# Hitenze/Preconditioned_Additive_Gaussian_Processes_with_Fourier_Acceleration

Hardware: AMD Instinct MI355X
Metric: kernel matvecs/sec + PCG wall-time to 1e-6, n=1e6 d=32 additive, 1/2/4/8 GPU (higher is better)
Workload: dtype f64; 1 GPU; additive NFFT matvec, n=1000000, d=32, 32 x 1-D windows, Gaussian f=1 l=1 mu=0.01 (BASELINE configs[2]); n=1000000, d=32, nwindows=32, parallelism=single

## Files before the change

preconditioned_additive_gaussian_processes_with_fourier_acceleration_amd/csrc/internal.h:

```cpp
#pragma once

#include <hip/hip_runtime.h>

#include <cstdint>
#include <memory>
#include <utility>
#include <string>
#include <vector>

#include "../../include/nfft4gp_amd.h"

namespace nfft4gp_amd {

constexpr int kNos = 64;
constexpr int kBand = 32;
constexpr int kM = 4;
constexpr int kTaps = 2 * kM + 2;
constexpr int kDeg = 7;
constexpr int kNC = kDeg + 1;
constexpr int kR = 16;
constexpr int kWave = 64;
constexpr int kPad = 32;
constexpr int kMaxBlock = 4096 - kPad;

// ... 135 lines not shown
   std::vector<double> comp_sigma;
   int kernel = 0;
   double f = 1.0, l = 1.0, mu = 0.0;
   double weight = 1.0;
   double diag = 1.0;
   int B = kMaxBlock, CG = 3, ngroups = 0, nblocks = 0;
   int rec = 5;
   int spread_variant = -1;
   int spread_fold = 1;
   bool det = false;
   double* d_hb = nullptr;
   int nparts = 0;
   DevLayout dl;
   double* d_part = nullptr;
   double* d_w = nullptr;
   double* d_wd = nullptr;
   double* d_H = nullptr;
   double* d_Hd = nullptr;
   double* d_C = nullptr;
   double* d_dot_part = nullptr;
   unsigned int* d_dot_ticket = nullptr;
   double* d_part2 = nullptr;
   double* d_gsum = nullptr;
   double* d_H2 = nullptr;
   double* d_xs = nullptr;
   double* d_ys = nullptr;
   MdPlan md;
   bool timing = false;
   hipEvent_t* kev = nullptr;
   double ms[3] = {0, 0, 0};
   long long cnt[3] = {0, 0, 0};
};

int upload_tap_coeffs();
int launch_spread(const AdditivePlan& P, const double* d_x, double* d_part, hipStream_t stream);
int launch_grid(const AdditivePlan& P, const double* d_part, int nparts, int grad, hipStream_t stream);
int launch_spread_grid(AdditivePlan& P, const double* d_x, int grad, hipStream_t stream);
int launch_grid_from_sum(const AdditivePlan& P, const double* d_gridsum, int grad, hipStream_t stream);
constexpr int kPeerInline = 8;
struct PeerArgs {
   char* const* bufs = nullptr;
   char* inl[kPeerInline] = {};
   char* own = nullptr;
   int world = 0;
   unsigned int epoch = 0;
   unsigned int* err = nullptr;
   long long slot_doubles = 0;
   long long spin = 0;
};
int launch_reduce_parts(const AdditivePlan& P, const double* d_part, double* d_gridsum, hipStream_t stream,
                        const PeerArgs* A = nullptr);
int launch_shard_finish_split(const AdditivePlan& P, const double* d_gridsum, double alpha, const double* d_x,
                              double beta, double* d_y, int S, hipStream_t stream, const PeerArgs* A = nullptr,
                              const double* d_part = nullptr);
int launch_peer_grid(const AdditivePlan& P, const PeerArgs& A, const double* d_part, hipStream_t stream);
int launch_peer_sum(const AdditivePlan& P, const PeerArgs& A, double* d_grid, hipStream_t stream);
int launch_interp(const AdditivePlan& P, int grad, double alpha, const double* d_x, double beta, double* d_y,
                  hipStream_t stream, double* d_dot = nullptr);
int launch_interp_blocks(const AdditivePlan& P, double alpha, const double* d_x, double beta, double* d_y, int b0,
                         int b1, hipStream_t stream);
int launch_matvec2(AdditivePlan& P, double alpha, const double* x0, const double* x1, double beta, double* y0,
                   double* y1, hipStream_t stream);
int pick_spread_variant(const AdditivePlan& P);
bool grid_atomic(const AdditivePlan& P);
int pick_interp_threads(const AdditivePlan& P);
bool pick_interp_hl(const AdditivePlan& P);
int pick_hl_slots(const AdditivePlan& P);
int pick_interp2_threads();
int additive_matvec_multi(void* str, int nv, double alpha, const double* const* X, double beta, double* const* Y);
int additive_matvec_dot(void* str, const double* d_x, double* d_y, double* d_dot);
AdditivePlan* additive_plan_of(void* str);
bool additive_fused_dot_ok(void* str);

struct NysDev {
   int n = 0, k = 0;
   double eta = 0.0;
   double* U = nullptr;
   float* Uf = nullptr;
   double* s = nullptr;
   double* w = nullptr;
   double* part = nullptr;
   int nblk = 0;
   double setup_ms[4] = {0.0, 0.0, 0.0, 0.0};
   std::vector<double> hs;
   bool grad = false;
   double f2 = 0.0;
   double *Kall = nullptr, *dU = nullptr, *G = nullptr, *Gt = nullptr, *GdKG = nullptr, *D = nullptr;
   double *vk = nullptr, *vn = nullptr;
};
void nys_free(NysDev* N);
constexpr int kNysRows = 2048;
// ... 158 lines not shown
```

preconditioned_additive_gaussian_processes_with_fourier_acceleration_amd/csrc/nfft_api.cpp:

```cpp
#include <dlfcn.h>
#include <hip/hip_runtime.h>

#include <array>
#include <algorithm>
#include <atomic>
#include <chrono>
#include <thread>
#include <cmath>
#include <cstdio>
#include <cstdlib>
#include <cstring>
#include <mutex>
#include <vector>

#include "internal.h"
#include "reduce.hpp"

using namespace nfft4gp_amd;

namespace nfft4gp_amd {

namespace {
std::recursive_mutex g_rand_mu;
int g_rand_depth = 0;
// ... 52 lines not shown
      ok = cnt > 0 ? 1 : 0;
   }
   return ok;
}

bool is_device_ptr(const void* p)
{
   if (!p) return false;
   hipPointerAttribute_t attr;
   hipError_t e = hipPointerGetAttributes(&attr, p);
   if (e != hipSuccess) {
      (void)hipGetLastError();
      return false;
   }
   return attr.type == hipMemoryTypeDevice || attr.type == hipMemoryTypeManaged;
}

}

namespace {

struct TimingRec {
   std::array<hipEvent_t, 6> ev;
};

struct PlanExt {
   AdditivePlan P;
   std::vector<TimingRec> pending;
   std::vector<TimingRec> pool;
};

struct SingleAdj {
   str_adj pub{};
   double sigma_pub = 0.0;
   nfft4gp_kernel* owner = nullptr;
   int dim = 1;
   int max_n = 0;
   std::vector<double> data;
   PlanExt* plan = nullptr;
};

void dfree(void* p)
{
   if (p) (void)hipFree(p);
}

// ... 8 lines not shown
   dfree(P.d_part);
   dfree(P.d_part2);
   dfree(P.d_H2);
   dfree(P.d_dot_part);
   dfree(P.d_dot_ticket);
   P.d_part2 = P.d_H2 = nullptr;
   P.d_part = nullptr;
   P.d_dot_part = nullptr;
   P.d_dot_ticket = nullptr;
}

void free_plan(PlanExt* E)
{
   if (!E) return;
   AdditivePlan& P = E->P;
   free_layout(P);
   md_free(P);
   dfree(P.d_w);
   dfree(P.d_wd);
   dfree(P.d_H);
   dfree(P.d_Hd);
   dfree(P.d_hb);
   dfree(P.d_gsum);
   dfree(P.d_C);
   dfree(P.d_xs);
   dfree(P.d_ys);
   for (auto& r : E->pending)
      for (auto e : r.ev) (void)hipEventDestroy(e);
   for (auto& r : E->pool)
      for (auto e : r.ev) (void)hipEventDestroy(e);
   delete E;
}

template <class T, class A>
int upload(T** dptr, const std::vector<T, A>& h)
{
   if (*dptr) {
      (void)hipFree(*dptr);
      *dptr = nullptr;
   }
   if (h.empty()) return 0;
   NFFT4GP_HIP_CHECK(hipMalloc((void**)dptr, sizeof(T) * h.size()));
   NFFT4GP_HIP_CHECK(hipMemcpy(*dptr, h.data(), sizeof(T) * h.size(), hipMemcpyHostToDevice));
   return 0;
}

// ... 35 lines not shown
{
   const int ng = P.n_global;
   RawVec<uint32_t> qc((size_t)P.nw * P.n);
   P.comp_scale.assign(P.nw, 1.0);
   P.comp_centre.assign(P.nw, 0.0);
   std::vector<double> xs;
   if (std::any_of(P.comp_dims.begin(), P.comp_dims.end(), [](int d) { return d != 1; })) {
      std::vector<std::vector<double>> xsc(P.nw);
      for (int c = 0; c < P.nw; c++) {
         const double* col = buffer + (size_t)c * ng * P.dw;
         P.comp_scale[c] = centre_and_scale(col, ng, P.comp_dims[c], xsc[c]);
         if (P.comp_scale[c] < 0.0) {
            fprintf(stderr, "nfft4gp_amd: all points of window %d coincide (radius 0); the reference's scaling "
                            "0.25/radius (nfft_interface.c:190) is undefined there.\n", c);
            return -1;
         }
      }
      if (md_build_points(P, xsc)) return -1;
      P.points_ready = true;
      return 0;
   }
   const auto t0 = std::chrono::steady_clock::now();
   std::atomic<int> next{0};
   auto work = [&]() {
      std::vector<double> xw;
      for (int c = next++; c < P.nw; c = next++) {
         const double* col = buffer + (size_t)c * ng * P.dw;
         P.comp_scale[c] = centre_and_scale(col, ng, 1, xw, &P.comp_centre[c]);
         if (P.comp_scale[c] < 0.0) continue;
         for (int j = 0; j < P.n; j++) qc[(size_t)c * P.n + j] = quantize(xw[(size_t)P.row_begin + j]);
      }
   };
   {
      const int nt = std::max(1, std::min({16, P.nw, (int)std::thread::hardware_concurrency()}));
      std::vector<std::thread> th;
      for (int t = 1; t < nt; t++) th.emplace_back(work);
      work();
      for (auto& t : th) t.join();
   }
   for (int c = 0; c < P.nw; c++)
      if (P.comp_scale[c] < 0.0) {
         fprintf(stderr,
                 "nfft4gp_amd: all points of window %d coincide (radius 0); the reference's scaling "
                 "0.25/radius (nfft_interface.c:190) is undefined there.\n", c);
         return -1;
      }
   const auto t1 = std::chrono::steady_clock::now();
   free_layout(P);
   hipStream_t s = current_stream();
   uint32_t* d_qc = nullptr;
   NFFT4GP_HIP_CHECK(hipMalloc((void**)&d_qc, sizeof(uint32_t) * std::max<size_t>(1, qc.size())));
   NFFT4GP_HIP_CHECK(hipMemcpyAsync(d_qc, qc.data(), sizeof(uint32_t) * qc.size(), hipMemcpyHostToDevice, s));
   const auto t2 = std::chrono::steady_clock::now();
   const int rc_dev = build_layout_dev(d_qc, P.n, P.nw, P.B, P.CG, P, s, P.rec);
   (void)hipStreamSynchronize(s);
   (void)hipFree(d_qc);
   if (rc_dev) {
      Layout L;
      build_layout(qc.data(), P.n, P.nw, P.B, P.CG, L, P.rec);
      P.ngroups = L.ngroups;
      P.nblocks = L.nblocks;
      free_layout(P);
      if (upload(&P.dl.meta, L.meta) || upload(&P.dl.lo, L.lo) || upload(&P.dl.q, L.q) ||
          upload(&P.dl.tile_off, L.tile_off) || upload(&P.dl.cmax, L.cmax))
         return -1;
      P.dl.ntiles = L.ntiles;
      P.dl.bytes = L.meta.size() * 2 + L.lo.size() * 4 + L.q.size() * 4 + L.tile_off.size() * 4;
   }
   if (getenv("NFFT4GP_AMD_VERBOSE")) {
// ... 45 lines not shown
      P.comp_sigma[c] = sig;
      bhat_1d(kernel == 0 ? 0 : 2, sig, bh);
      bhat_1d(kernel == 0 ? 1 : 3, sig, bhd);
      const double dscale = (kernel == 0) ? 2.0 * sc * std::sqrt(2.0) / sig : sc / sig;
      circulant_1d(bh, P.weight, w.data() + (size_t)c * kNos);
      circulant_1d(bhd, P.weight * dscale, wd.data() + (size_t)c * kNos);
   }
   if (upload(&P.d_w, w) || upload(&P.d_wd, wd)) return -1;
   return 0;
}

TimingRec get_rec(PlanExt* E)
{
   if (!E->pool.empty()) {
      TimingRec r = E->pool.back();
      E->pool.pop_back();
      return r;
   }
   TimingRec r;
   for (auto& e : r.ev) (void)hipEventCreate(&e);
   return r;
}

int plan_apply_dev(PlanExt* E, int grad, double alpha, const double* d_x, double beta, double* d_y)
{
   AdditivePlan& P = E->P;
   hipStream_t s = current_stream();
   TimingRec rec;
   if (P.timing) {
      rec = get_rec(E);
      if (!P.md.on) P.kev = rec.ev.data();
   }
   const bool mdt = P.timing && P.md.on;
   int rc = 0;
   if (mdt) (void)hipEventRecord(rec.ev[0], s);
   if (P.md.on) {
      rc = md_spread(P, d_x, P.md.d_grid, s);
      if (mdt) {
         (void)hipEventRecord(rec.ev[1], s);
         (void)hipEventRecord(rec.ev[2], s);
      }
      if (!rc) rc = md_grid(P, P.md.d_grid, grad, s);
   } else {
      rc = launch_spread_grid(P, d_x, grad, s);
   }
   if (mdt) {
      (void)hipEventRecord(rec.ev[3], s);
      (void)hipEventRecord(rec.ev[4], s);
   }
   if (!rc)
      rc = P.md.on ? md_interp(P, grad, alpha, d_x, beta, d_y, s) : launch_interp(P, grad, alpha, d_x, beta, d_y, s);
   if (mdt) (void)hipEventRecord(rec.ev[5], s);
   P.kev = nullptr;
   if (P.timing) {
      if (rc)
         E->pool.push_back(rec);
      else
         E->pending.push_back(rec);
   }
   return rc ? -1 : 0;
}

int plan_apply(PlanExt* E, int n, int grad, double alpha, const double* x, double beta, double* y)
{
   AdditivePlan& P = E->P;
   if (!P.points_ready) {
      fprintf(stderr, "nfft4gp_amd: matvec called before the kernel setup (func_kernel) call.\n");
      return -1;
   }
   if (n != P.n) {
      fprintf(stderr, "nfft4gp_amd: matvec size %d does not match the handle (%d).\n", n, P.n);
      return -1;
   }
// ... 76 lines not shown
{
   P.B = default_block(P.n);
   {
      const int nw = std::max(P.nw, 1), nblocks = std::max(1, (P.n + P.B - 1) / P.B);
      auto pick = [&](int cgmax) {
         const int ngroups = (nw + cgmax - 1) / cgmax;
         P.CG = (nw + ngroups - 1) / ngroups;
         return ngroups;
      };
      if ((long long)pick(4) * nblocks < 384) pick(3);
   }
   if (const char* e = getenv("NFFT4GP_AMD_BLOCK")) {
      const int v = atoi(e);
      if (v >= 256) P.B = std::min(v, kMaxBlock) & ~15;
   }
   if (const char* e = getenv("NFFT4GP_AMD_CG")) {
      const int v = atoi(e);
      if (v >= 1 && v <= 64) P.CG = v;
   }
   if (const char* e = getenv("NFFT4GP_AMD_SPREAD_VARIANT")) P.spread_variant = atoi(e);
   if (const char* e = getenv("NFFT4GP_AMD_SPREAD_FOLD")) P.spread_fold = atoi(e) != 0;
   if (const char* e = getenv("NFFT4GP_AMD_DET")) P.det = atoi(e) != 0;
   if (const char* e = getenv("NFFT4GP_AMD_PRECISION")) P.rec = atoi(e) == 32 ? 4 : 5;
}

void* additive_create(double* data, int n_global, int ldim, int d, int* windows, int nwindows, int dwindows, int rb,
                      int re)
{
   nfft4gp_kernel* kd = kernel_struct_create(3 * n_global);
   kd->_iparams[0] = nwindows;
   kd->_iparams[1] = dwindows;
   int skip_window = 1;
   kd->_iparams[2] = 0;
   while (skip_window < dwindows && windows[nwindows * dwindows - skip_window] < 0) {
      skip_window++;
      kd->_iparams[2]++;
   }
   kd->_ibufferp = (int**)malloc(sizeof(int*));
   kd->_ibufferp[0] = windows;
   kd->_buffer = (double*)malloc(sizeof(double) * (size_t)n_global * nwindows * dwindows);
   kd->_own_buffer = 1;
   PlanExt* E = new PlanExt();
   AdditivePlan& P = E->P;
   P.n_global = n_global;
   P.row_begin = rb;
   P.row_end = re;
// ... 26 lines not shown

}

namespace nfft4gp_amd {
bool additive_fused_dot_ok(void* str)
{
   PlanExt* E = additive_plan(str);
   if (!E || !E->P.points_ready) return false;
   const AdditivePlan& P = E->P;
   if (P.row_begin != 0 || P.row_end != P.n_global) return false;
   return P.md.on || P.nblocks <= kRedMaxBlocks;
}

int additive_matvec_dot(void* str, const double* d_x, double* d_y, double* d_dot)
{
   PlanExt* E = additive_plan(str);
   if (!E || !E->P.points_ready) return -1;
   AdditivePlan& P = E->P;
   hipStream_t s = current_stream();
   if (P.md.on) {
      if (md_spread(P, d_x, P.md.d_grid, s) || md_grid(P, P.md.d_grid, 0, s)) return -1;
      return md_interp(P, 0, 1.0, d_x, 0.0, d_y, s, d_dot);
   }
   if (launch_spread_grid(P, d_x, 0, s)) return -1;
   return launch_interp(P, 0, 1.0, d_x, 0.0, d_y, s, d_dot);
}
}

namespace nfft4gp_amd {
int additive_matvec_multi(void* str, int nv, double alpha, const double* const* X, double beta, double* const* Y)
{
   PlanExt* E = additive_plan(str);
   if (!E || !E->P.points_ready) return -1;
   AdditivePlan& P = E->P;
   if (P.row_begin != 0 || P.row_end != P.n_global) return -1;
   hipStream_t s = current_stream();
   int v = 0;
   if (!P.md.on && !P.timing)
      for (; v + 1 < nv; v += 2)
         if (launch_matvec2(P, alpha, X[v], X[v + 1], beta, Y[v], Y[v + 1], s)) return -1;
   for (; v < nv; v++)
      if (plan_apply_dev(E, 0, alpha, X[v], beta, Y[v])) return -1;
   return 0;
}

int additive_matvec_chunked(void* str, double alpha, const double* d_x, double* d_y, int nchunks,
// ... 231 lines not shown
void Nfft4GPAdditiveNFFTKernelFree(void* str)
{
   if (!str) return;
   free_plan(additive_plan(str));
   ((nfft4gp_kernel*)str)->_external = NULL;
   Nfft4GPKernelParamFree(str);
}

double* Nfft4GPNFFTAppendData(double* X1, int n1, int ldim1, int d, double* X2, int n2, int ldim2)
{
   double* X = (double*)malloc(sizeof(double) * (size_t)(n1 + n2) * d);
   for (int i = 0; i < d; i++) {
      memcpy(X + (size_t)i * (n1 + n2), X1 + (size_t)i * ldim1, sizeof(double) * n1);
      memcpy(X + (size_t)i * (n1 + n2) + n1, X2 + (size_t)i * ldim2, sizeof(double) * n2);
   }
   return X;
}

int Nfft4GPAmdAdditiveLayoutInfo(void* str, long long* out, int nout)
{
   PlanExt* E = additive_plan(str);
   if (!E || !out) return -1;
   const AdditivePlan& P = E->P;
   long long v[16] = {P.n, P.nw, P.B, P.nblocks, P.dl.ntiles, P.dl.ntiles * kWave * kR, kR, P.CG, P.ngroups,
                      (long long)P.dl.bytes, pick_spread_variant(P), grid_atomic(P), pick_interp_threads(P),
                      pick_interp_hl(P), pick_hl_slots(P), pick_interp2_threads()};
   for (int i = 0; i < nout && i < 16; i++) out[i] = v[i];
   return 0;
}

int Nfft4GPAmdSetPrecision(void* str, int bits)
{
   PlanExt* E = additive_plan(str);
   if (!E || (bits != 32 && bits != 64)) {
      fprintf(stderr, "nfft4gp_amd: Nfft4GPAmdSetPrecision needs an additive handle and bits 32 or 64\n");
      return -1;
   }
   AdditivePlan& P = E->P;
   const int rec = bits == 32 ? 4 : 5;
   if (rec == P.rec) return 0;
   (void)hipStreamSynchronize(current_stream());
   P.rec = rec;
   if (!P.points_ready || P.md.on) return 0;
   const double* buffer = ((nfft4gp_kernel*)str)->_buffer;
   P.points_ready = false;
   if (plan_build_points(P, buffer)) return -1;
   return plan_setup(P, buffer, P.kernel, P.f, P.l, P.mu);
}

int Nfft4GPAmdSetDeterministic(void* str, int on)
// ... 10 lines not shown
   PlanExt* E = additive_plan(str);
   if (!E) return -1;
   E->P.timing = enable != 0;
   if (enable) {
      (void)hipStreamSynchronize(current_stream());
      for (auto& r : E->pending) E->pool.push_back(r);
      E->pending.clear();
      for (int i = 0; i < 3; i++) {
         E->P.ms[i] = 0;
         E->P.cnt[i] = 0;
      }
   }
   return 0;
}

int Nfft4GPAmdTimingQuery(void* str, double* ms, long long* cnt)
{
   PlanExt* E = additive_plan(str);
   if (!E) return -1;
   AdditivePlan& P = E->P;
   for (auto& r : E->pending) {
      NFFT4GP_HIP_CHECK(hipEventSynchronize(r.ev[5]));
      for (int i = 0; i < 3; i++) {
         float t = 0.f;
         NFFT4GP_HIP_CHECK(hipEventElapsedTime(&t, r.ev[2 * i], r.ev[2 * i + 1]));
         P.ms[i] += t;
         P.cnt[i]++;
      }
      E->pool.push_back(r);
   }
   E->pending.clear();
   for (int i = 0; i < 3; i++) {
      if (ms) ms[i] = P.ms[i];
      if (cnt) cnt[i] = P.cnt[i];
   }
   return 0;
}

int Nfft4GPAmdKernelBench(void* str, int which, int grad, int reps, const double* x, double* y, double* ms_avg)
{
   PlanExt* E = additive_plan(str);
   if (!E || !E->P.points_ready || reps <= 0 || !ms_avg) return -1;
   AdditivePlan& P = E->P;
   if (!is_device_ptr(x) || !is_device_ptr(y)) {
      fprintf(stderr, "nfft4gp_amd: Nfft4GPAmdKernelBench needs device vectors\n");
      return -1;
// ... 311 lines not shown
```

preconditioned_additive_gaussian_processes_with_fourier_acceleration_amd/csrc/nfft_kernels.hip:

```cpp
#include <hip/hip_ext.h>
#include <hip/hip_runtime.h>

#include <algorithm>
#include <cmath>
#include <cstdio>
#include <vector>

#include "internal.h"
#include "reduce.hpp"

namespace nfft4gp_amd {

constexpr int kGridThreads = 1024;
constexpr int kMomStride = kNC + 1;
constexpr int kMomWin = kNC * kNos + 4;
template <int MOMT>
__host__ __device__ constexpr int mom_doubles_per_window()
{
   return MOMT ? kMomWin : kNos * kMomStride;
}
template <int MOMT>
__device__ __forceinline__ int mom_index(int cl, int cell, int d)
{
   return MOMT ? cl * kMomWin + d * kNos + cell : (cl * kNos + cell) * kMomStride + d;
// ... 141 lines not shown
   for (int ks = 0; ks < 2; ks++)
#pragma unroll
      for (int cb = 0; cb < 4; cb++) bm[ks][cb] = mrow[(4 * ks + k) * kNos + 16 * cb + i];
#pragma unroll
   for (int cb = 0; cb < 4; cb++) {
      f64x4 acc = {0.0, 0.0, 0.0, 0.0};
      acc = __builtin_amdgcn_mfma_f64_16x16x4f64(a[0], bm[0][cb], acc, 0, 0, 0);
      acc = __builtin_amdgcn_mfma_f64_16x16x4f64(a[1], bm[1][cb], acc, 0, 0, 0);
      mrow[k * kNos + 16 * cb + i] = acc[0];
      mrow[(4 + k) * kNos + 16 * cb + i] = acc[1];
      if (k < kTaps - 8) grow89[k * kNos + 16 * cb + i] = acc[2];
   }
   __builtin_amdgcn_fence(__ATOMIC_RELEASE, "wavefront");
   __builtin_amdgcn_wave_barrier();
   __builtin_amdgcn_fence(__ATOMIC_ACQUIRE, "wavefront");
   double v = 0.0;
#pragma unroll
   for (int tp = 0; tp < kTaps; tp++) {
      const int cell = (lane + kM - tp) & (kNos - 1);
      v += tp < 8 ? mrow[tp * kNos + cell] : grow89[(tp - 8) * kNos + cell];
   }
   return v;
}

template <int THREADS, bool TIMELINE = false, int MOMT = 1, bool DET = false, int REC = 5, bool PIPE = false>
__global__ __launch_bounds__(THREADS, 6) void k_spread(const uint16_t* __restrict__ meta,
                                                      const uint32_t* __restrict__ lo,
                                                      const uint32_t* __restrict__ qarr,
                                                      const int* __restrict__ tile_off, const int* __restrict__ cmax,
                                                      const double* __restrict__ x, int n, int B, int nblocks,
                                                      int ngroups, int CG, int nw, double* __restrict__ part,
                                                      double* __restrict__ gsum, int fold)
{
   extern __shared__ __attribute__((aligned(16))) double smem[];
   const int Bp = B + kPad;
   double* s_alpha = smem;
   double* s_mom = smem + Bp;
   uint32_t* s_red = reinterpret_cast<uint32_t*>(s_mom + CG * mom_doubles_per_window<MOMT>());

   const int xcd = blockIdx.x & 7;
   const int rest = blockIdx.x >> 3;
   const int g = rest % ngroups;
   const int b = (rest / ngroups) * 8 + xcd;
   if (b >= nblocks) return;
   if (TIMELINE) stamp(0);

// ... 686 lines not shown
      if (t + nwaves < t1) load_tile<REC>(cur, meta, lo, qarr, t + nwaves, lane);
   }
   for (; g < ngroups; g++) leave(g);
   __syncthreads();

   const double ff = f * f;
#pragma unroll
   for (int k = 0; k < kEpMax; k++) {
      if (!ep_regs) break;
      const int j = tid + k * THREADS;
      if (j >= nloc) break;
      const double v = ff * (s_y[j] + mu * xe[k]);
      y[(size_t)base + j] = (beta == 0.0) ? alpha * v : fma(beta, ye[k], alpha * v);
   }
   if (!ep_regs) {
      for (int j = tid; j < nloc; j += THREADS) {
         const size_t gj = (size_t)base + j;
         const double v = ff * (s_y[j] + mu * x[gj]);
         y[gj] = (beta == 0.0) ? alpha * v : fma(beta, y[gj], alpha * v);
      }
   }
}


template <int THREADS, bool DET = false, int REC = 5>
__global__ __launch_bounds__(THREADS) void k_interp2(const uint16_t* __restrict__ meta,
                                                     const uint32_t* __restrict__ lo,
                                                     const uint32_t* __restrict__ qarr,
                                                     const int* __restrict__ tile_off, const double* __restrict__ H,
                                                     size_t h_rs, const double* __restrict__ x0,
                                                     const double* __restrict__ x1, double* __restrict__ y0,
                                                     double* __restrict__ y1, int n, int B, int ngroups, double alpha,
                                                     double beta, double f, double mu, const double* __restrict__ hb,
                                                     int nw)
{
   extern __shared__ __attribute__((aligned(16))) double smem[];
   const int Bp = B + kPad;
   double* s_y0 = smem;
   double* s_y1 = smem + Bp;
   const int b = blockIdx.x;
   const int tid = threadIdx.x;
   const int base = b * B;
   const int nloc = min(B, n - base);
   const int lane = tid & 63;
   const int wave = tid >> 6;
   constexpr int nwaves = THREADS / 64;
// ... 129 lines not shown
static InterpFn interp_fn(bool grad, bool dot, bool small, bool det, int rec)
{
   if (rec == 4) return small ? interp_fn_t<512, 4>(grad, dot, det) : interp_fn_t<kInterpThreads, 4>(grad, dot, det);
   return small ? interp_fn_t<512, 5>(grad, dot, det) : interp_fn_t<kInterpThreads, 5>(grad, dot, det);
}
constexpr int kInterp2Threads = 1024;
typedef void (*Interp2Fn)(const uint16_t*, const uint32_t*, const uint32_t*, const int*, const double*, size_t,
                          const double*, const double*, double*, double*, int, int, int, double, double, double, double,
                          const double*, int);
template <int REC>
static Interp2Fn interp2_fn_t(bool det, bool small)
{
   if (small) return det ? k_interp2<512, true, REC> : k_interp2<512, false, REC>;
   return det ? k_interp2<kInterp2Threads, true, REC> : k_interp2<kInterp2Threads, false, REC>;
}
static Interp2Fn interp2_fn(bool det, bool small, int rec)
{
   return rec == 4 ? interp2_fn_t<4>(det, small) : interp2_fn_t<5>(det, small);
}
typedef void (*InterpPartFn)(const uint16_t*, const uint32_t*, const uint32_t*, const int*, const double*, double*, int,
                             int, int, int, double);
static InterpPartFn interp_part_fn(int rec) { return rec == 4 ? k_interp_part<512, 4> : k_interp_part<512, 5>; }

static bool static_lds_zero(const void* fn)
{
   hipFuncAttributes a;
   if (hipFuncGetAttributes(&a, fn) != hipSuccess) return false;
   return a.sharedSizeBytes == 0;
}

typedef void (*InterpHlFn)(const uint16_t*, const uint32_t*, const uint32_t*, const int*, const double*, const double*,
                           double*, int, int, int, int, int, double, double, double, double, const double*, int);
static InterpHlFn interp_hl_fn(bool small, bool det, int rec)
{
   if (rec == 4)
      return small ? (det ? k_interp_hl<512, true, 4> : k_interp_hl<512, false, 4>)
                   : (det ? k_interp_hl<1024, true, 4> : k_interp_hl<1024, false, 4>);
   return small ? (det ? k_interp_hl<512, true, 5> : k_interp_hl<512, false, 5>)
                : (det ? k_interp_hl<1024, true, 5> : k_interp_hl<1024, false, 5>);
}
bool pick_interp_hl(const AdditivePlan& P)
{
   static const int v = getenv("NFFT4GP_AMD_INTERP_HL") ? atoi(getenv("NFFT4GP_AMD_INTERP_HL")) : -1;
   return (v < 0 ? P.dl.bytes > kInfinityCacheBytes : v != 0) && P.ngroups >= 1;
}
int pick_interp_threads(const AdditivePlan& P)
// ... 9 lines not shown
   return ns;
}
int pick_interp2_threads()
{
   static const int forced = getenv("NFFT4GP_AMD_INTERP2_THREADS") ? atoi(getenv("NFFT4GP_AMD_INTERP2_THREADS")) : 0;
   return forced == 512 ? 512 : kInterp2Threads;
}

static std::vector<const void*> interp_kernels()
{
   std::vector<const void*> v;
   for (int sm = 0; sm < 2; sm++)
      for (int det = 0; det < 2; det++)
         for (int rec = 4; rec <= 5; rec++) v.push_back((const void*)interp_hl_fn(sm, det, rec));
   for (int g = 0; g < 2; g++)
      for (int d = 0; d < 2; d++)
         for (int sm = 0; sm < 2; sm++)
            for (int det = 0; det < 2; det++)
               for (int rec = 4; rec <= 5; rec++) v.push_back((const void*)interp_fn(g, d && !g, sm, det, rec));
   for (int det = 0; det < 2; det++)
      for (int sm = 0; sm < 2; sm++)
         for (int rec = 4; rec <= 5; rec++) v.push_back((const void*)interp2_fn(det, sm, rec));
   for (int rec = 4; rec <= 5; rec++) v.push_back((const void*)interp_part_fn(rec));
   return v;
}

static void raise_lds_limit_once()
{
   static const bool raised = []() {
      for (const auto& byrec : kSpreadFns)
         for (const auto& bydet : byrec)
            for (const SpreadFn f : bydet)
               (void)hipFuncSetAttribute((const void*)f, hipFuncAttributeMaxDynamicSharedMemorySize, (int)kMaxDynamicLds);
      for (const void* f : interp_kernels())
         (void)hipFuncSetAttribute(f, hipFuncAttributeMaxDynamicSharedMemorySize, (int)kMaxDynamicLds);
      (void)hipGetLastError();
      return true;
   }();
   (void)raised;
}

static bool abs_lds_ok()
{
   static const bool ok = [] {
      std::vector<const void*> v = interp_kernels();
      for (const auto& byrec : kSpreadFns)
         for (const auto& bydet : byrec)
            for (const SpreadFn f : bydet) v.push_back((const void*)f);
      for (const void* f : v)
         if (!static_lds_zero(f)) return false;
      return true;
   }();
   if (!ok) fprintf(stderr, "nfft4gp_amd: a matvec kernel has static LDS; its absolute LDS addressing would be wrong\n");
   return ok;
}

static int launch_spread_to(const AdditivePlan& P, const double* d_x, double* d_part, double* d_gsum,
                            hipStream_t stream)
{
   if (P.dl.ntiles == 0 || P.n == 0) return 0;
   raise_lds_limit_once();
   if (!abs_lds_ok()) return -1;
   const SpreadFn fn = spread_fn(P);
   const int gridx = ((P.nblocks + 7) / 8) * 8 * P.ngroups;
   launch_ev(fn, dim3(gridx), dim3(kSpreadThreads), spread_lds_bytes(P), stream, P.kev ? P.kev + 0 : nullptr,
             P.dl.meta, P.dl.lo, P.dl.q, P.dl.tile_off, (const int*)P.dl.cmax, d_x, P.n, P.B, P.nblocks, P.ngroups,
             P.CG, P.nw, d_part, d_gsum, P.spread_fold);
   NFFT4GP_HIP_CHECK(hipGetLastError());
   return 0;
}

// ... 101 lines not shown
   if (P.n == 0) return 0;
   raise_lds_limit_once();
   if (!abs_lds_ok()) return -1;
   if (d_dot && (grad || P.nblocks > kRedMaxBlocks)) {
      fprintf(stderr, "nfft4gp_amd: fused matvec-dot needs a plain matvec and <= %d blocks\n", kRedMaxBlocks);
      return -1;
   }
   const bool small = pick_interp_threads(P) == 512;
   if (!grad && !d_dot && pick_interp_hl(P)) {
      const int ns = pick_hl_slots(P);
      launch_ev(interp_hl_fn(small, P.det, P.rec), dim3(P.nblocks), dim3(small ? 512 : kInterpThreads),
                hl_lds_bytes(P.B, P.CG, P.ngroups, ns), stream, P.kev ? P.kev + 4 : nullptr, P.dl.meta, P.dl.lo,
                P.dl.q, P.dl.tile_off, (const double*)P.d_H, d_x, d_y, P.n, P.B, P.ngroups, P.CG, P.nw, alpha, beta,
                P.f, P.mu * P.diag, (const double*)P.d_hb, ns);
      NFFT4GP_HIP_CHECK(hipGetLastError());
      return 0;
   }
   const InterpFn fn = interp_fn(grad, d_dot != nullptr, small, P.det, P.rec);
   launch_ev(fn, dim3(P.nblocks), dim3(small ? 512 : kInterpThreads), interp_lds_bytes(P, grad), stream,
             P.kev ? P.kev + 4 : nullptr, P.dl.meta, P.dl.lo, P.dl.q, P.dl.tile_off, (const double*)P.d_H,
             (const double*)P.d_Hd, d_x, d_y, P.n, P.B, P.ngroups, alpha, beta, P.f, P.mu * P.diag, P.diag,
             P.d_dot_part, P.d_dot_ticket, d_dot, (const double*)P.d_hb, P.nw);
   NFFT4GP_HIP_CHECK(hipGetLastError());
   return 0;
}

int launch_interp_blocks(const AdditivePlan& P, double alpha, const double* d_x, double beta, double* d_y, int b0,
                         int b1, hipStream_t stream)
{
   if (P.n == 0 || b1 <= b0) return 0;
   raise_lds_limit_once();
   if (!abs_lds_ok()) return -1;
   const size_t off = (size_t)b0 * P.B;
   hipLaunchKernelGGL(interp_fn(false, false, false, P.det, P.rec), dim3(b1 - b0), dim3(kInterpThreads),
                      interp_lds_bytes(P, 0), stream, P.dl.meta, P.dl.lo, P.dl.q, P.dl.tile_off + (size_t)b0 * P.ngroups,
                      (const double*)P.d_H, (const double*)P.d_Hd, d_x + off, d_y + off, P.n - (int)off, P.B, P.ngroups,
                      alpha, beta, P.f, P.mu * P.diag, P.diag, (double*)nullptr, (unsigned int*)nullptr,
                      (double*)nullptr, (const double*)P.d_hb, P.nw);
   NFFT4GP_HIP_CHECK(hipGetLastError());
   return 0;
}

int launch_matvec2(AdditivePlan& P, double alpha, const double* x0, const double* x1, double beta, double* y0,
                   double* y1, hipStream_t stream)
{
   if (P.n == 0) return 0;
// ... 23 lines not shown
```

preconditioned_additive_gaussian_processes_with_fourier_acceleration_amd/nfft.py:

```python
from __future__ import annotations

import ctypes as C

import numpy as np

from . import _lib

GAUSSIAN = 0
MATERN12 = 1


def _ptr(a):
    if isinstance(a, np.ndarray):
        if not a.flags.c_contiguous or a.dtype != np.float64:
            raise ValueError("numpy vectors must be C-contiguous float64")
        return a.ctypes.data, False
    if not a.is_contiguous() or str(a.dtype) != "torch.float64":
        raise ValueError("torch vectors must be contiguous float64")
    return a.data_ptr(), a.is_cuda


def _numel(a) -> int:
    return int(a.size) if isinstance(a, np.ndarray) else int(a.numel())

# ... 117 lines not shown
            raise RuntimeError("shard spread failed")
        return grid

    def shard_grid_size(self) -> int:
        return int(_lib.lib().Nfft4GPAmdShardGridSize(self.h))

    def shard_finish(self, grid, x_local, alpha=1.0, beta=0.0, y_local=None, grad=False):
        _check_len("x_local", x_local, self.n)
        if y_local is None:
            y_local = _empty_like(x_local, (3 if grad else 1) * self.n)
        _check_len("y_local", y_local, (3 if grad else 1) * self.n)
        size = self.shard_grid_size()
        if size < 0:
            raise RuntimeError("run the kernel setup before shard_finish")
        _check_len("grid", grid, size, exact=False)
        gp, _ = _ptr(grid)
        xp, _ = _ptr(x_local)
        yp, _ = _ptr(y_local)
        if _lib.lib().Nfft4GPAmdShardFinish(self.h, gp, int(grad), float(alpha), xp, float(beta), yp) != 0:
            raise RuntimeError("shard finish failed")
        return y_local

    def layout_info(self) -> dict:
        out = (C.c_longlong * 16)()
        _lib.lib().Nfft4GPAmdAdditiveLayoutInfo(self.h, out, 16)
        keys = ["n", "nwindows", "block", "nblocks", "ntiles", "slots", "R", "comps_per_group", "ngroups",
                "layout_bytes", "spread_variant", "grid_atomic", "interp_threads", "interp_hl", "hl_slots",
                "interp2_threads"]
        return dict(zip(keys, [int(v) for v in out]))

    def set_deterministic(self, on: bool = True):
        if _lib.lib().Nfft4GPAmdSetDeterministic(self.h, int(bool(on))) != 0:
            raise RuntimeError("Nfft4GPAmdSetDeterministic failed")

    def set_precision(self, bits: int):
        if _lib.lib().Nfft4GPAmdSetPrecision(self.h, int(bits)) != 0:
            raise RuntimeError("Nfft4GPAmdSetPrecision failed")

    def timing(self, enable: bool):
        _lib.lib().Nfft4GPAmdTimingEnable(self.h, int(enable))

    def timing_query(self):
        ms = (C.c_double * 3)()
        cnt = (C.c_longlong * 3)()
        _lib.lib().Nfft4GPAmdTimingQuery(self.h, ms, cnt)
        names = ["spread", "grid", "interp"]
        return {nm: (ms[i], int(cnt[i])) for i, nm in enumerate(names)}

    KERNELS = ("spread", "grid", "interp")

    def kernel_bench(self, kernel: str, x, y, reps: int = 50, grad: bool = False) -> float:
# ... 90 lines not shown
```

Measured before the change: 14360 matvecs/s.

## Fuse grid circulant stage into interpolation kernel with double-buffered grid sums

```diff
diff --git a/preconditioned_additive_gaussian_processes_with_fourier_acceleration_amd/csrc/internal.h b/preconditioned_additive_gaussian_processes_with_fourier_acceleration_amd/csrc/internal.h
--- a/preconditioned_additive_gaussian_processes_with_fourier_acceleration_amd/csrc/internal.h
+++ b/preconditioned_additive_gaussian_processes_with_fourier_acceleration_amd/csrc/internal.h
@@ -181,6 +181,10 @@
    unsigned int* d_dot_ticket = nullptr;
    double* d_part2 = nullptr;
    double* d_gsum = nullptr;
+   int fused_grid = -1;
+   bool cells33 = false;
+   double* d_hsum = nullptr;
+   int hsum_par = 0;
    double* d_H2 = nullptr;
    double* d_xs = nullptr;
    double* d_ys = nullptr;
@@ -226,6 +230,9 @@
 bool pick_interp_hl(const AdditivePlan& P);
 int pick_hl_slots(const AdditivePlan& P);
 int pick_interp2_threads();
+bool pick_fused_grid(const AdditivePlan& P);
+int launch_matvec_fused(AdditivePlan& P, double alpha, const double* d_x, double beta, double* d_y, hipStream_t stream,
+                        double* d_dot = nullptr);
 int additive_matvec_multi(void* str, int nv, double alpha, const double* const* X, double beta, double* const* Y);
 int additive_matvec_dot(void* str, const double* d_x, double* d_y, double* d_dot);
 AdditivePlan* additive_plan_of(void* str);
diff --git a/preconditioned_additive_gaussian_processes_with_fourier_acceleration_amd/csrc/nfft_api.cpp b/preconditioned_additive_gaussian_processes_with_fourier_acceleration_amd/csrc/nfft_api.cpp
--- a/preconditioned_additive_gaussian_processes_with_fourier_acceleration_amd/csrc/nfft_api.cpp
+++ b/preconditioned_additive_gaussian_processes_with_fourier_acceleration_amd/csrc/nfft_api.cpp
@@ -98,6 +98,7 @@
 
 struct TimingRec {
    std::array<hipEvent_t, 6> ev;
+   bool grid = true;
 };
 
 struct PlanExt {
@@ -152,6 +153,7 @@
    dfree(P.d_Hd);
    dfree(P.d_hb);
    dfree(P.d_gsum);
+   dfree(P.d_hsum);
    dfree(P.d_C);
    dfree(P.d_xs);
    dfree(P.d_ys);
@@ -233,13 +235,20 @@
    }
    const auto t0 = std::chrono::steady_clock::now();
    std::atomic<int> next{0};
+   std::atomic<int> outside33{0};
    auto work = [&]() {
       std::vector<double> xw;
       for (int c = next++; c < P.nw; c = next++) {
          const double* col = buffer + (size_t)c * ng * P.dw;
          P.comp_scale[c] = centre_and_scale(col, ng, 1, xw, &P.comp_centre[c]);
          if (P.comp_scale[c] < 0.0) continue;
-         for (int j = 0; j < P.n; j++) qc[(size_t)c * P.n + j] = quantize(xw[(size_t)P.row_begin + j]);
+         uint32_t cimax = 0;
+         for (int j = 0; j < P.n; j++) {
+            const uint32_t q = quantize(xw[(size_t)P.row_begin + j]);
+            qc[(size_t)c * P.n + j] = q;
+            cimax = std::max(cimax, (q + 0x40000000u) >> 26);
+         }
+         if (cimax > 32u) outside33 = 1;
       }
    };
    {
@@ -256,6 +265,7 @@
                  "0.25/radius (nfft_interface.c:190) is undefined there.\n", c);
          return -1;
       }
+   P.cells33 = outside33 == 0;
    const auto t1 = std::chrono::steady_clock::now();
    free_layout(P);
    hipStream_t s = current_stream();
@@ -347,6 +357,17 @@
    return r;
 }
 
+bool use_fused(const AdditivePlan& P, hipStream_t s)
+{
+   if (!pick_fused_grid(P)) return false;
+   hipStreamCaptureStatus st = hipStreamCaptureStatusNone;
+   if (hipStreamIsCapturing(s, &st) != hipSuccess) {
+      (void)hipGetLastError();
+      return false;
+   }
+   return st == hipStreamCaptureStatusNone;
+}
+
 int plan_apply_dev(PlanExt* E, int grad, double alpha, const double* d_x, double beta, double* d_y)
 {
    AdditivePlan& P = E->P;
@@ -359,6 +380,8 @@
    const bool mdt = P.timing && P.md.on;
    int rc = 0;
    if (mdt) (void)hipEventRecord(rec.ev[0], s);
+   const bool fused = !grad && use_fused(P, s);
+   rec.grid = !fused;
    if (P.md.on) {
       rc = md_spread(P, d_x, P.md.d_grid, s);
       if (mdt) {
@@ -366,6 +389,8 @@
          (void)hipEventRecord(rec.ev[2], s);
       }
       if (!rc) rc = md_grid(P, P.md.d_grid, grad, s);
+   } else if (fused) {
+      rc = launch_matvec_fused(P, alpha, d_x, beta, d_y, s);
    } else {
       rc = launch_spread_grid(P, d_x, grad, s);
    }
@@ -373,7 +398,7 @@
       (void)hipEventRecord(rec.ev[3], s);
       (void)hipEventRecord(rec.ev[4], s);
    }
-   if (!rc)
+   if (!rc && !fused)
       rc = P.md.on ? md_interp(P, grad, alpha, d_x, beta, d_y, s) : launch_interp(P, grad, alpha, d_x, beta, d_y, s);
    if (mdt) (void)hipEventRecord(rec.ev[5], s);
    P.kev = nullptr;
@@ -496,6 +521,7 @@
    if (const char* e = getenv("NFFT4GP_AMD_SPREAD_FOLD")) P.spread_fold = atoi(e) != 0;
    if (const char* e = getenv("NFFT4GP_AMD_DET")) P.det = atoi(e) != 0;
    if (const char* e = getenv("NFFT4GP_AMD_PRECISION")) P.rec = atoi(e) == 32 ? 4 : 5;
+   if (const char* e = getenv("NFFT4GP_AMD_FUSED_GRID")) P.fused_grid = atoi(e) != 0;
 }
 
 void* additive_create(double* data, int n_global, int ldim, int d, int* windows, int nwindows, int dwindows, int rb,
@@ -568,6 +594,7 @@
       if (md_spread(P, d_x, P.md.d_grid, s) || md_grid(P, P.md.d_grid, 0, s)) return -1;
       return md_interp(P, 0, 1.0, d_x, 0.0, d_y, s, d_dot);
    }
+   if (use_fused(P, s)) return launch_matvec_fused(P, 1.0, d_x, 0.0, d_y, s, d_dot);
    if (launch_spread_grid(P, d_x, 0, s)) return -1;
    return launch_interp(P, 0, 1.0, d_x, 0.0, d_y, s, d_dot);
 }
@@ -845,10 +872,10 @@
    PlanExt* E = additive_plan(str);
    if (!E || !out) return -1;
    const AdditivePlan& P = E->P;
-   long long v[16] = {P.n, P.nw, P.B, P.nblocks, P.dl.ntiles, P.dl.ntiles * kWave * kR, kR, P.CG, P.ngroups,
+   long long v[17] = {P.n, P.nw, P.B, P.nblocks, P.dl.ntiles, P.dl.ntiles * kWave * kR, kR, P.CG, P.ngroups,
                       (long long)P.dl.bytes, pick_spread_variant(P), grid_atomic(P), pick_interp_threads(P),
-                      pick_interp_hl(P), pick_hl_slots(P), pick_interp2_threads()};
-   for (int i = 0; i < nout && i < 16; i++) out[i] = v[i];
+                      pick_interp_hl(P), pick_hl_slots(P), pick_interp2_threads(), pick_fused_grid(P)};
+   for (int i = 0; i < nout && i < 17; i++) out[i] = v[i];
    return 0;
 }
 
@@ -905,6 +932,7 @@
    for (auto& r : E->pending) {
       NFFT4GP_HIP_CHECK(hipEventSynchronize(r.ev[5]));
       for (int i = 0; i < 3; i++) {
+         if (i == 1 && !r.grid) continue;
          float t = 0.f;
          NFFT4GP_HIP_CHECK(hipEventElapsedTime(&t, r.ev[2 * i], r.ev[2 * i + 1]));
          P.ms[i] += t;
diff --git a/preconditioned_additive_gaussian_processes_with_fourier_acceleration_amd/csrc/nfft_kernels.hip b/preconditioned_additive_gaussian_processes_with_fourier_acceleration_amd/csrc/nfft_kernels.hip
--- a/preconditioned_additive_gaussian_processes_with_fourier_acceleration_amd/csrc/nfft_kernels.hip
+++ b/preconditioned_additive_gaussian_processes_with_fourier_acceleration_amd/csrc/nfft_kernels.hip
@@ -187,6 +187,10 @@
    }
    return v;
 }
+
+constexpr int kFgCells = 33;
+constexpr int kFgSpan = kFgCells + kTaps - 1;
+constexpr int kFgSpan0 = (kNos - 16 - kM) & (kNos - 1);
 
 template <int THREADS, bool TIMELINE = false, int MOMT = 1, bool DET = false, int REC = 5, bool PIPE = false>
 __global__ __launch_bounds__(THREADS, 6) void k_spread(const uint16_t* __restrict__ meta,
@@ -919,6 +923,161 @@
    }
 }
 
+constexpr int kFgWin = kNC * kFgCells + 1;
+constexpr int kFgRow = kNos + 1;
+constexpr int kFgQuads = (kFgSpan + 3) / 4;
+constexpr int kFgHs = 4 * kFgQuads + 1;
+constexpr int kFgLdsWin = kFgWin + kFgHs + 2 * kFgRow;
+
+template <int THREADS, bool DOT = false, int REC = 5>
+__global__ __launch_bounds__(THREADS) void k_interp_fg(
+    const uint16_t* __restrict__ meta, const uint32_t* __restrict__ lo, const uint32_t* __restrict__ qarr,
+    const int* __restrict__ tile_off, const double* __restrict__ gsum, double* __restrict__ gclear,
+    const double* __restrict__ wcirc, const double* __restrict__ x, double* __restrict__ y, int n, int B, int ngroups,
+    double alpha, double beta, double f, double mu, double* __restrict__ dot_part,
+    unsigned int* __restrict__ dot_ticket, double* __restrict__ dot_out, int nw)
+{
+   static_assert(THREADS % (4 * kNC) == 0 && kNC == 8, "a thread keeps its degree and cell quarter over the build");
+   static_assert(kFgSpan % 6 == 0, "the circulant's steps go six per trip");
+   extern __shared__ __attribute__((aligned(16))) double smem[];
+   const int Bp = B + kPad;
+   double* s_y = smem;
+   double* s_H = smem + Bp;
+   double* s_h = s_H + (size_t)nw * kFgWin;
+   double* s_g = s_h + (size_t)nw * kFgHs;
+   double* s_w = s_g + (size_t)nw * kFgRow;
+   double* s_scr = s_w + (size_t)nw * kFgRow;
+   const int b = blockIdx.x;
+   const int tid = threadIdx.x;
+   const int base = b * B;
+   const int nloc = min(B, n - base);
+   const int lane = tid & 63;
+   const int wave = tid >> 6;
+   constexpr int nwaves = THREADS / 64;
+   const int t0 = tile_off[b * ngroups];
+   const int t1 = tile_off[(b + 1) * ngroups];
+   TileRegs cur;
+   int t = t0 + wave;
+   if (t < t1) load_tile<REC>(cur, meta, lo, qarr, t, lane);
+   double ct[kTaps];
+#pragma unroll
+   for (int tp = 0; tp < kTaps; tp++) ct[tp] = c_taps[tp * kNC + (tid & (kNC - 1))];
+   for (int i = tid; i < nw * kNos; i += THREADS) {
+      const int o = (i >> 6) * kFgRow + (i & (kNos - 1));
+      s_g[o] = gsum[i];
+      s_w[o] = wcirc[i];
+   }
+   if (b == 0)
+      for (int i = tid; i < nw * kNos; i += THREADS) gclear[i] = 0.0;
+   for (int i = tid; i < Bp; i += THREADS) s_y[i] = 0.0;
+   __syncthreads();
+   for (int it = tid; it < nw * kFgQuads; it += THREADS) {
+      const int w = it / kFgQuads, k0 = 4 * (it % kFgQuads);
+      const double* gw = s_g + w * kFgRow;
+      const double* ww = s_w + w * kFgRow;
+      double r3 = ww[(k0 + 3) & (kNos - 1)], r2 = ww[(k0 + 2) & (kNos - 1)], r1 = ww[(k0 + 1) & (kNos - 1)], r0 = ww[k0];
+      double a0 = 0.0, a1 = 0.0, a2 = 0.0, a3 = 0.0;
+#pragma unroll 6
+      for (int j = 0; j < kFgSpan; j++) {
+         const double gj = gw[(kFgSpan0 + j) & (kNos - 1)];
+         a0 = fma(r0, gj, a0);
+         a1 = fma(r1, gj, a1);
+         a2 = fma(r2, gj, a2);
+         a3 = fma(r3, gj, a3);
+         r3 = r2, r2 = r1, r1 = r0;
+         r0 = ww[(k0 - j - 1) & (kNos - 1)];
+      }
+      double* hw = s_h + w * kFgHs + k0;
+      hw[0] = a0, hw[1] = a1, hw[2] = a2, hw[3] = a3;
+   }
+   __syncthreads();
+   {
+      const int d = tid & (kNC - 1), seg = (tid >> 3) & 3;
+      const int c0 = seg ? 8 * seg + 1 : 0, c1 = 8 * seg + 9;
+      for (int w = tid >> 5; w < nw; w += THREADS / 32) {
+         const double* hw = s_h + w * kFgHs + c0;
+         double hv[kTaps + 8];
+#pragma unroll
+         for (int j = 0; j < kTaps + 8; j++) hv[j] = hw[j];
+         double acc[9];
+#pragma unroll
+         for (int k = 0; k < 9; k++) acc[k] = 0.0;
+#pragma unroll
+         for (int tp = 0; tp < kTaps; tp++) {
+#pragma unroll
+            for (int k = 0; k < 9; k++) acc[k] = fma(hv[k + tp], ct[tp], acc[k]);
+         }
+         double* dst = s_H + (size_t)w * kFgWin + d * kFgCells + c0;
+#pragma unroll
+         for (int k = 0; k < 9; k++)
+            if (c0 + k < c1) dst[k] = acc[k];
+      }
+   }
+   __syncthreads();
+   const bool ep_regs = B <= kEpMax * THREADS;
+   double xe[kEpMax], ye[kEpMax];
+   if (ep_regs) {
+#pragma unroll
+      for (int k = 0; k < kEpMax; k++) {
+         const int j = tid + k * THREADS;
+         xe[k] = (j < nloc) ? x[(size_t)base + j] : 0.0;
+         ye[k] = (beta != 0.0 && j < nloc) ? y[(size_t)base + j] : 0.0;
+      }
+   }
+
+   for (; t < t1; t += nwaves) {
+      const int tn = t + nwaves;
+      const int ci = min((int)((cur.mt + 16u) & 63u), kFgCells - 1);
+      const double* hrow = s_H + (size_t)(cur.mt >> 6) * kFgWin + ci;
+      double hc[kNC];
+#pragma unroll
+      for (int d = 0; d < kNC; d++) hc[d] = hrow[d * kFgCells];
+#pragma unroll
+      for (int r = 0; r < kR; r++) {
+         const uint32_t off = slot_off<REC>(cur, r);
+         const double u = q_to_s(cur.qq[r]);
+         double v = hc[kNC - 1];
+#pragma unroll
+         for (int d = kNC - 2; d >= 0; d--) v = fma(v, u, hc[d]);
+         lds_add(off, v);
+      }
+      if (tn < t1) load_tile<REC>(cur, meta, lo, qarr, tn, lane);
+   }
+   __syncthreads();
+
+   const double ff = f * f;
+   double dacc = 0.0;
+#pragma unroll
+   for (int k = 0; k < kEpMax; k++) {
+      if (!ep_regs) break;
+      const int j = tid + k * THREADS;
+      if (j >= nloc) break;
+      const double xj = xe[k];
+      const double v = ff * (s_y[j] + mu * xj);
+      const double yo = (beta == 0.0) ? alpha * v : fma(beta, ye[k], alpha * v);
+      y[(size_t)base + j] = yo;
+      if (DOT) dacc = fma(yo, xj, dacc);
+   }
+   if (!ep_regs) {
+      for (int j = tid; j < nloc; j += THREADS) {
+         const size_t gj = (size_t)base + j;
+         const double xj = x[gj];
+         const double v = ff * (s_y[j] + mu * xj);
+         const double yo = (beta == 0.0) ? alpha * v : fma(beta, y[gj], alpha * v);
+         y[gj] = yo;
+         if (DOT) dacc = fma(yo, xj, dacc);
+      }
+   }
+   if (DOT) {
+      dacc = block_sum0_s<THREADS>(dacc, s_scr);
+      double tot;
+      if (grid_total_s<THREADS>(dacc, dot_part, dot_ticket, &tot, reinterpret_cast<int*>(s_scr + 2 * (THREADS / 64)),
+                                s_scr + THREADS / 64) &&
+          threadIdx.x == 0)
+         *dot_out = tot;
+   }
+}
+
 
 template <int THREADS, bool DET = false, int REC = 5>
 __global__ __launch_bounds__(THREADS) void k_interp2(const uint16_t* __restrict__ meta,
@@ -1094,6 +1253,15 @@
                              int, int, int, double);
 static InterpPartFn interp_part_fn(int rec) { return rec == 4 ? k_interp_part<512, 4> : k_interp_part<512, 5>; }
 
+typedef void (*InterpFgFn)(const uint16_t*, const uint32_t*, const uint32_t*, const int*, const double*, double*,
+                           const double*, const double*, double*, int, int, int, double, double, double, double,
+                           double*, unsigned int*, double*, int);
+static InterpFgFn interp_fg_fn(bool dot, int rec)
+{
+   if (rec == 4) return dot ? k_interp_fg<kInterpThreads, true, 4> : k_interp_fg<kInterpThreads, false, 4>;
+   return dot ? k_interp_fg<kInterpThreads, true, 5> : k_interp_fg<kInterpThreads, false, 5>;
+}
+
 static bool static_lds_zero(const void* fn)
 {
    hipFuncAttributes a;
@@ -1149,16 +1317,24 @@
       for (int sm = 0; sm < 2; sm++)
          for (int rec = 4; rec <= 5; rec++) v.push_back((const void*)interp2_fn(det, sm, rec));
    for (int rec = 4; rec <= 5; rec++) v.push_back((const void*)interp_part_fn(rec));
+   for (int d = 0; d < 2; d++)
+      for (int rec = 4; rec <= 5; rec++) v.push_back((const void*)interp_fg_fn(d, rec));
    return v;
 }
+static std::vector<const void*> spread_kernels()
+{
+   std::vector<const void*> v;
+   for (const auto& byrec : kSpreadFns)
+      for (const auto& bydet : byrec)
+         for (const SpreadFn f : bydet) v.push_back((const void*)f);
+   return v;
+}
 
 static void raise_lds_limit_once()
 {
    static const bool raised = []() {
-      for (const auto& byrec : kSpreadFns)
-         for (const auto& bydet : byrec)
-            for (const SpreadFn f : bydet)
-               (void)hipFuncSetAttribute((const void*)f, hipFuncAttributeMaxDynamicSharedMemorySize, (int)kMaxDynamicLds);
+      for (const void* f : spread_kernels())
+         (void)hipFuncSetAttribute(f, hipFuncAttributeMaxDynamicSharedMemorySize, (int)kMaxDynamicLds);
       for (const void* f : interp_kernels())
          (void)hipFuncSetAttribute(f, hipFuncAttributeMaxDynamicSharedMemorySize, (int)kMaxDynamicLds);
       (void)hipGetLastError();
@@ -1171,9 +1347,7 @@
 {
    static const bool ok = [] {
       std::vector<const void*> v = interp_kernels();
-      for (const auto& byrec : kSpreadFns)
-         for (const auto& bydet : byrec)
-            for (const SpreadFn f : bydet) v.push_back((const void*)f);
+      for (const void* f : spread_kernels()) v.push_back(f);
       for (const void* f : v)
          if (!static_lds_zero(f)) return false;
       return true;
@@ -1321,6 +1495,44 @@
              (const double*)P.d_Hd, d_x, d_y, P.n, P.B, P.ngroups, alpha, beta, P.f, P.mu * P.diag, P.diag,
              P.d_dot_part, P.d_dot_ticket, d_dot, (const double*)P.d_hb, P.nw);
    NFFT4GP_HIP_CHECK(hipGetLastError());
+   return 0;
+}
+
+static size_t fg_lds_bytes(int B, int nw)
+{
+   return sizeof(double) * ((size_t)B + kPad) + sizeof(double) * (size_t)nw * kFgLdsWin + kRedScratch;
+}
+constexpr int kFusedMaxBlocks = 256;
+bool pick_fused_grid(const AdditivePlan& P)
+{
+   if (P.fused_grid == 0 || !P.cells33 || P.md.on || P.det || P.nblocks == 0 || P.n == 0) return false;
+   if (P.row_begin != 0 || P.row_end != P.n_global) return false;
+   if (!grid_atomic(P) || pick_interp_threads(P) != kInterpThreads || pick_interp_hl(P)) return false;
+   if (fg_lds_bytes(P.B, P.nw) > kMaxDynamicLds) return false;
+   return P.fused_grid > 0 || P.nblocks <= kFusedMaxBlocks;
+}
+
+int launch_matvec_fused(AdditivePlan& P, double alpha, const double* d_x, double beta, double* d_y, hipStream_t stream,
+                        double* d_dot)
+{
+   raise_lds_limit_once();
+   if (!abs_lds_ok()) return -1;
+   if (d_dot && P.nblocks > kRedMaxBlocks) return -1;
+   const size_t ns = (size_t)P.nw * kNos;
+   if (!P.d_hsum) {
+      NFFT4GP_HIP_CHECK(hipMalloc((void**)&P.d_hsum, sizeof(double) * 2 * ns));
+      NFFT4GP_HIP_CHECK(hipMemsetAsync(P.d_hsum, 0, sizeof(double) * 2 * ns, stream));
+      P.hsum_par = 0;
+   }
+   double* S = P.d_hsum + (size_t)P.hsum_par * ns;
+   double* Sother = P.d_hsum + (size_t)(1 - P.hsum_par) * ns;
+   if (launch_spread_to(P, d_x, nullptr, S, stream)) return -1;
+   launch_ev(interp_fg_fn(d_dot != nullptr, P.rec), dim3(P.nblocks), dim3(kInterpThreads), fg_lds_bytes(P.B, P.nw),
+             stream, P.kev ? P.kev + 4 : nullptr, P.dl.meta, P.dl.lo, P.dl.q, P.dl.tile_off, (const double*)S, Sother,
+             (const double*)P.d_w, d_x, d_y, P.n, P.B, P.ngroups, alpha, beta, P.f, P.mu * P.diag, P.d_dot_part,
+             P.d_dot_ticket, d_dot, P.nw);
+   NFFT4GP_HIP_CHECK(hipGetLastError());
+   P.hsum_par ^= 1;
    return 0;
 }
 
diff --git a/preconditioned_additive_gaussian_processes_with_fourier_acceleration_amd/nfft.py b/preconditioned_additive_gaussian_processes_with_fourier_acceleration_amd/nfft.py
--- a/preconditioned_additive_gaussian_processes_with_fourier_acceleration_amd/nfft.py
+++ b/preconditioned_additive_gaussian_processes_with_fourier_acceleration_amd/nfft.py
@@ -163,11 +163,11 @@
         return y_local
 
     def layout_info(self) -> dict:
-        out = (C.c_longlong * 16)()
-        _lib.lib().Nfft4GPAmdAdditiveLayoutInfo(self.h, out, 16)
+        out = (C.c_longlong * 17)()
+        _lib.lib().Nfft4GPAmdAdditiveLayoutInfo(self.h, out, 17)
         keys = ["n", "nwindows", "block", "nblocks", "ntiles", "slots", "R", "comps_per_group", "ngroups",
                 "layout_bytes", "spread_variant", "grid_atomic", "interp_threads", "interp_hl", "hl_slots",
-                "interp2_threads"]
+                "interp2_threads", "fused_grid"]
         return dict(zip(keys, [int(v) for v in out]))
 
     def set_deterministic(self, on: bool = True):
```

Measured after the change: 14820 matvecs/s, median of 6. 1.03x the previous value.
